# gdalsanto/flamo

Measured on AMD Instinct MI355X. Metric: freq-bin*channel products/sec (fwd+bwd), nfft=96000 8x8ch, higher is better.
Workload: dtype f32; 1 GPU; BASELINE configs[1]: Shell(FFT -> Series(Matrix 8x8, GEQ 8x8) -> iFFT), nfft=96000, batch 32 per GPU, fwd+bwd of (y**2).mean(), parameter grads; nfft=96000, channels=8, batch_per_gpu=32, parallelism=dp1 (batch), input_grad=False

## Files before the change

### flamo_amd/csrc/fusedfwd.hip

```cpp
#include "spectral_common.h"
#include "spec_cols_body.h"
#include "fusedfwd.h"

namespace fl {
using namespace sp32;

template <int A, int B, int VT, int RG, bool PLAIN, int NIW>
__global__ void __launch_bounds__(256, 5) cols_fwd_rc_kernel(ColsArgs a, RcBaArgs r, int n_mix, int n_rc, int rc_gx, long long* dbg) {
    extern __shared__ __attribute__((aligned(16))) char smem[];
    const int i = blockIdx.x;
    int role = 0;
    if (dbg && threadIdx.x == 0) dbg[4 * (size_t)i] = (long long)__builtin_amdgcn_s_memrealtime();
    if (i >= n_mix) {
        spec_cols_fwd_body<A, B, VT, RG, PLAIN>(a, i - n_rc, smem);
    } else {
        const int before = (int)(((long)i * n_rc) / n_mix), after = (int)(((long)(i + 1) * n_rc) / n_mix);
        if (after > before) {
            role = 1;
            rc_ba_body<NIW>(r, before % rc_gx, before / rc_gx, smem);
        } else {
            spec_cols_fwd_body<A, B, VT, RG, PLAIN>(a, i - before, smem);
        }
    }
    if (dbg && threadIdx.x == 0) {
        dbg[4 * (size_t)i + 1] = (long long)__builtin_amdgcn_s_memrealtime();
        dbg[4 * (size_t)i + 2] = role;
        dbg[4 * (size_t)i + 3] = (long long)__builtin_amdgcn_s_getreg((31 << 11) | 4) | ((long long)__builtin_amdgcn_s_getreg((31 << 11) | 20) << 32);
    }
}

static void pin_kernel_order() {
    (void)&cols_fwd_rc_kernel<8, 25, 16, 1, true, 8>, (void)&cols_fwd_rc_kernel<8, 25, 16, 1, true, 4>,
        (void)&cols_fwd_rc_kernel<8, 25, 16, 1, false, 8>, (void)&cols_fwd_rc_kernel<8, 25, 16, 1, false, 4>;
}

static thread_local bool t_pair_mode = false, t_have = false;
static thread_local PendingRc t_pending;
static long long* g_pair_dbg = nullptr;
static long g_pair_launches = 0;
static int g_pair_density = [] { const char* e = getenv("FLAMO_PAIR_DENSITY"); return e ? atoi(e) : 140; }();
static int g_pair_enabled = [] { const char* e = getenv("FLAMO_LAUNCH_PAIR"); return e ? atoi(e) : 1; }();

long long* pair_dbg() { return g_pair_dbg; }
bool pair_mode() { return t_pair_mode && g_pair_enabled; }
void pending_rc_put(const PendingRc& p) {
    t_pending = p;
    t_have = true;
}
bool pending_rc_take(PendingRc& out) {
    if (!t_have) return false;
    out = t_pending;
    t_have = false;
    return true;
}

int fused_cols_rc_launch(const ColsArgs& a, unsigned n_cols, const PendingRc& rc, hipStream_t st) {
    const int vt = a.CT << a.cgs;
    if (a.L1 != 200 || vt != 16 || !(rc.niw == 8 || rc.niw == 4)) return FL_ERR_UNSUPPORTED;
    constexpr int A = 8, B = 25, LEN = A * B, LENP = LEN | 1;
    size_t lds = ((size_t)16 * LENP + LEN + (size_t)16 * B) * sizeof(cf);
    if (rc.lds > lds) lds = rc.lds;
    const long n_rc = (long)rc.gx * rc.gy, total = (long)n_cols + n_rc;
    if (total >= (1l << 31)) return FL_ERR_UNSUPPORTED;
    const bool plain = a.env_log2 == 0.0 && a.t_lim >= a.n;
    long n_mix = n_rc + (long)n_cols * 100 / (g_pair_density > 0 ? g_pair_density : 100);
    if (n_mix > total) n_mix = total;
    if (n_mix < n_rc) n_mix = n_rc;
    RcBaArgs rargs = rc.args;
    rargs.dbg = g_pair_dbg ? g_pair_dbg + 4 * 8192 : nullptr;
    dispatch<1, 0>(plain, [&](auto PLAIN) {
        dispatch<8, 4>(rc.niw, [&](auto NIW) {
            hipLaunchKernelGGL((cols_fwd_rc_kernel<A, B, 16, 1, decltype(PLAIN)::value != 0, decltype(NIW)::value>), dim3((unsigned)total), dim3(256),
                               lds, st, a, rargs, (int)n_mix, (int)n_rc, rc.gx, g_pair_dbg);
        });
    });
    FL_CHECK_LAUNCH("cols_fwd_rc");
    ++g_pair_launches;
    return FL_OK;
}

}

using namespace fl;

extern "C" {

int fl_launch_pair_begin(void) {
    if (t_have) {
        set_error("launch pair: begin while a recorded response launch is pending (flush it first)");
        return FL_ERR_BAD_ARG;
    }
    t_pair_mode = true;
    return FL_OK;
}

int fl_launch_pair_pending(void) { return t_have ? 1 : 0; }

long fl_debug_launch_pair_count(void) { return g_pair_launches; }

int fl_debug_set_pair_stamps(void* buf) {
    g_pair_dbg = (long long*)buf;
    return FL_OK;
}

int fl_launch_pair_flush(void* stream) {
    t_pair_mode = false;
    PendingRc p;
    if (pending_rc_take(p)) return rc_ba_launch_now(p, (hipStream_t)stream);
    return FL_OK;
}

}
```

Baseline: 666.5 billion products/s.

## Replace interleaved grid with persistent work-queue kernel for cols and response tiles

```diff
diff --git a/flamo_amd/csrc/fusedfwd.hip b/flamo_amd/csrc/fusedfwd.hip
--- a/flamo_amd/csrc/fusedfwd.hip
+++ b/flamo_amd/csrc/fusedfwd.hip
@@ -5,27 +5,96 @@
 namespace fl {
 using namespace sp32;
 
-template <int A, int B, int VT, int RG, bool PLAIN, int NIW>
-__global__ void __launch_bounds__(256, 5) cols_fwd_rc_kernel(ColsArgs a, RcBaArgs r, int n_mix, int n_rc, int rc_gx, long long* dbg) {
-    extern __shared__ __attribute__((aligned(16))) char smem[];
-    const int i = blockIdx.x;
-    int role = 0;
-    if (dbg && threadIdx.x == 0) dbg[4 * (size_t)i] = (long long)__builtin_amdgcn_s_memrealtime();
-    if (i >= n_mix) {
-        spec_cols_fwd_body<A, B, VT, RG, PLAIN>(a, i - n_rc, smem);
-    } else {
-        const int before = (int)(((long)i * n_rc) / n_mix), after = (int)(((long)(i + 1) * n_rc) / n_mix);
-        if (after > before) {
-            role = 1;
-            rc_ba_body<NIW>(r, before % rc_gx, before / rc_gx, smem);
+constexpr int kColHeads = 8, kRcHead = kColHeads, kTicket = kColHeads + 1, kQueueWords = 12;
+__device__ unsigned g_pair_queue[kQueueWords];
+constexpr unsigned kNoTile = 0xffffffffu;
+
+__device__ __forceinline__ unsigned q_pop(int w) { return __hip_atomic_fetch_add(&g_pair_queue[w], 1u, __ATOMIC_RELAXED, __HIP_MEMORY_SCOPE_AGENT); }
+__device__ __forceinline__ unsigned q_peek(int w) { return __hip_atomic_load(&g_pair_queue[w], __ATOMIC_RELAXED, __HIP_MEMORY_SCOPE_AGENT); }
+
+__device__ __forceinline__ unsigned pair_next_tile(int pref, int xcd, int n_cols, int n_rc, bool& scan) {
+    if (!scan) {
+        if (pref) {
+            const unsigned k = q_pop(kRcHead);
+            if (k < (unsigned)n_rc) return (unsigned)n_cols + k;
         } else {
-            spec_cols_fwd_body<A, B, VT, RG, PLAIN>(a, i - before, smem);
+            const unsigned k = q_pop(xcd);
+            if ((unsigned long long)k * kColHeads + xcd < (unsigned long long)n_cols) return k * kColHeads + xcd;
+        }
+        scan = true;
+    }
+    for (;;) {
+        unsigned head[kColHeads + 1];
+#pragma unroll
+        for (int w = 0; w <= kColHeads; ++w) head[w] = q_peek(w);
+        int pick = -1;
+        if (pref && head[kRcHead] < (unsigned)n_rc) pick = kRcHead;
+#pragma unroll
+        for (int d = 0; d < kColHeads; ++d) {
+            const int w = (xcd + d) & (kColHeads - 1);
+            if (pick < 0 && (unsigned long long)head[w] * kColHeads + w < (unsigned long long)n_cols) pick = w;
+        }
+        if (pick < 0 && head[kRcHead] < (unsigned)n_rc) pick = kRcHead;
+        if (pick < 0) return kNoTile;
+        const unsigned k = q_pop(pick);
+        if (pick == kRcHead) {
+            if (k < (unsigned)n_rc) return (unsigned)n_cols + k;
+        } else if ((unsigned long long)k * kColHeads + pick < (unsigned long long)n_cols) {
+            return k * kColHeads + pick;
         }
     }
-    if (dbg && threadIdx.x == 0) {
-        dbg[4 * (size_t)i + 1] = (long long)__builtin_amdgcn_s_memrealtime();
-        dbg[4 * (size_t)i + 2] = role;
-        dbg[4 * (size_t)i + 3] = (long long)__builtin_amdgcn_s_getreg((31 << 11) | 4) | ((long long)__builtin_amdgcn_s_getreg((31 << 11) | 20) << 32);
+}
+
+__global__ void pair_queue_snapshot(unsigned* out) {
+    for (int w = 0; w < kQueueWords; ++w) out[w] = q_peek(w);
+}
+
+struct PairArgs {
+    ColsArgs a;
+    RcBaArgs r;
+    int n_cols, n_rc, rc_gx, resp_keys;
+    long long* dbg;
+};
+
+typedef const __attribute__((address_space(4))) PairArgs* PairArgsPtr;
+
+template <int NIW>
+__device__ __attribute__((noinline)) void pair_rc_tile(PairArgsPtr kp, int k, char* smem) {
+    const PairArgs& p = *(const PairArgs*)kp;
+    rc_ba_body<NIW>(p.r, k % p.rc_gx, k / p.rc_gx, smem);
+}
+
+template <int A, int B, int VT, int RG, bool PLAIN, int NIW>
+__global__ void __launch_bounds__(256, 5) cols_fwd_rc_kernel(PairArgs) {
+    extern __shared__ __attribute__((aligned(16))) char smem[];
+    __shared__ unsigned s_tile;
+    const PairArgsPtr kp = (PairArgsPtr)__builtin_amdgcn_kernarg_segment_ptr();
+    const unsigned hw = __builtin_amdgcn_s_getreg((31 << 11) | 4), xcc = __builtin_amdgcn_s_getreg((31 << 11) | 20);
+    const int xcd = (int)(xcc & (kColHeads - 1));
+    const int key = (int)((hw >> 8) & 0xf) * 4 + (int)((hw >> 13) & 0x3);
+    const int pref = key < kp->resp_keys ? 1 : 0;
+    const int n_cols = kp->n_cols, n_rc = kp->n_rc;
+    long long* dbg = kp->dbg;
+    bool scan = false;
+    for (;;) {
+        if (threadIdx.x == 0) s_tile = pair_next_tile(pref, xcd, n_cols, n_rc, scan);
+        __syncthreads();
+        const unsigned t = __builtin_amdgcn_readfirstlane(s_tile);
+        if (t == kNoTile) break;
+        const bool stamp = dbg && threadIdx.x == 0 && t < 8192u;
+        if (stamp) dbg[4 * (size_t)t] = (long long)__builtin_amdgcn_s_memrealtime();
+        if (t < (unsigned)n_cols) spec_cols_fwd_body<A, B, VT, RG, PLAIN>(((const PairArgs*)kp)->a, (int)t, smem);
+        else pair_rc_tile<NIW>(kp, (int)t - n_cols, smem);
+        if (stamp) {
+            dbg[4 * (size_t)t + 1] = (long long)__builtin_amdgcn_s_memrealtime();
+            dbg[4 * (size_t)t + 2] = (long long)(t < (unsigned)n_cols ? 0 : 1) | ((long long)blockIdx.x << 32);
+            dbg[4 * (size_t)t + 3] = (long long)hw | ((long long)xcc << 32);
+        }
+        __syncthreads();
+    }
+    if (threadIdx.x == 0 && q_pop(kTicket) == gridDim.x - 1) {
+#pragma unroll
+        for (int w = 0; w < kQueueWords; ++w) __hip_atomic_store(&g_pair_queue[w], 0u, __ATOMIC_RELAXED, __HIP_MEMORY_SCOPE_AGENT);
     }
 }
 
@@ -38,8 +107,8 @@
 static thread_local PendingRc t_pending;
 static long long* g_pair_dbg = nullptr;
 static long g_pair_launches = 0;
-static int g_pair_density = [] { const char* e = getenv("FLAMO_PAIR_DENSITY"); return e ? atoi(e) : 140; }();
 static int g_pair_enabled = [] { const char* e = getenv("FLAMO_LAUNCH_PAIR"); return e ? atoi(e) : 1; }();
+constexpr int kPairResponseCus = 128;
 
 long long* pair_dbg() { return g_pair_dbg; }
 bool pair_mode() { return t_pair_mode && g_pair_enabled; }
@@ -54,6 +123,14 @@
     return true;
 }
 
+static int pair_response_cus(int cus) {
+    const char* e = getenv("FLAMO_PAIR_RESPONSE_CUS");
+    int R = e && *e ? atoi(e) : kPairResponseCus;
+    if (R < 0) R = 0;
+    if (R > cus) R = cus;
+    return R & ~7;
+}
+
 int fused_cols_rc_launch(const ColsArgs& a, unsigned n_cols, const PendingRc& rc, hipStream_t st) {
     const int vt = a.CT << a.cgs;
     if (a.L1 != 200 || vt != 16 || !(rc.niw == 8 || rc.niw == 4)) return FL_ERR_UNSUPPORTED;
@@ -63,17 +140,22 @@
     const long n_rc = (long)rc.gx * rc.gy, total = (long)n_cols + n_rc;
     if (total >= (1l << 31)) return FL_ERR_UNSUPPORTED;
     const bool plain = a.env_log2 == 0.0 && a.t_lim >= a.n;
-    long n_mix = n_rc + (long)n_cols * 100 / (g_pair_density > 0 ? g_pair_density : 100);
-    if (n_mix > total) n_mix = total;
-    if (n_mix < n_rc) n_mix = n_rc;
+    const int cus = device_cus();
+    const long grid = total < 5l * cus ? total : 5l * cus;
+    const int R = pair_response_cus(cus), per_xcd = cus / 8 > 0 ? cus / 8 : 1, ids = 4 * (per_xcd / 4 + 1);
+    const int resp_keys = R >= cus ? 64 : (R / 8 * ids + per_xcd - 1) / per_xcd;
     RcBaArgs rargs = rc.args;
     rargs.dbg = g_pair_dbg ? g_pair_dbg + 4 * 8192 : nullptr;
+    unsigned* qrec = g_pair_dbg ? reinterpret_cast<unsigned*>(g_pair_dbg + 4 * 8192 + 8 * 8 * 4096) : nullptr;
+    if (qrec) pair_queue_snapshot<<<1, 1, 0, st>>>(qrec);
+    const PairArgs pargs = {a, rargs, (int)n_cols, (int)n_rc, rc.gx, resp_keys, g_pair_dbg};
     dispatch<1, 0>(plain, [&](auto PLAIN) {
         dispatch<8, 4>(rc.niw, [&](auto NIW) {
-            hipLaunchKernelGGL((cols_fwd_rc_kernel<A, B, 16, 1, decltype(PLAIN)::value != 0, decltype(NIW)::value>), dim3((unsigned)total), dim3(256),
-                               lds, st, a, rargs, (int)n_mix, (int)n_rc, rc.gx, g_pair_dbg);
+            hipLaunchKernelGGL((cols_fwd_rc_kernel<A, B, 16, 1, decltype(PLAIN)::value != 0, decltype(NIW)::value>), dim3((unsigned)grid), dim3(256),
+                               lds, st, pargs);
         });
     });
+    if (qrec) pair_queue_snapshot<<<1, 1, 0, st>>>(qrec + kQueueWords);
     FL_CHECK_LAUNCH("cols_fwd_rc");
     ++g_pair_launches;
     return FL_OK;
```

New measurement: 397.6 billion products/s. 0.596x the previous value.
